# gylien/scale-letkf

Measured on AMD Instinct MI355X. Metric: grid-point LETKF solves/sec, higher is better.
Workload: dtype f64

## Files before the change

scale-letkf_amd/csrc/letkf_wave_dev.h:

```cpp
#pragma once
#include <hip/hip_runtime.h>
#include <stdint.h>

#include <type_traits>

#include "letkf_device.h"
#include "letkf_search_dev.h"
#include "letkf_jacobi_dev.h"
#include "letkf_lane_dev.h"
#include "letkf_sched_dev.h"

namespace letkf {

using namespace jacobi_dev;
using namespace lane_dev;

template <int NW, int OP>
__device__ __forceinline__ double preduce(double v, double* red, int& slot) {
  v = (OP == 0) ? wave_sum(v) : (OP == 1) ? wave_max(v) : wave_min(v);
  if constexpr (NW == 1) {
    return v;
  } else {
    if ((threadIdx.x & 63) == 0) red[2 * slot + (threadIdx.x >> 6)] = v;
    __syncthreads();
// ... 424 lines not shown
  if (NW == 1 && KR <= 50 && tot < 32 * KR + 64 * ((KR + 3) / 4) + 128)
    tot = 32 * KR + 64 * ((KR + 3) / 4) + 128;
  return (tot + 1) & ~1;
}

#ifdef LETKF_WAVE_PROF
#define PROF_DECL unsigned long long prof_t[10] = {0, 0, 0, 0, 0, 0, 0, 0, 0, 0}; unsigned long long prof_last = __builtin_amdgcn_s_memtime(); const unsigned long long prof_t0 = prof_last; int prof_units = 0;
#define PROF_MARK(i) { const unsigned long long t_ = __builtin_amdgcn_s_memtime(); prof_t[i] += t_ - prof_last; prof_last = t_; }
#define PROF_FLUSH if (A.prof && wlane == 0) { for (int i_ = 0; i_ < 10; ++i_) atomicAdd(&A.prof[i_], prof_t[i_]); \
    atomicMax(&A.prof[10], ~prof_t0); atomicMax(&A.prof[11], (unsigned long long)__builtin_amdgcn_s_memtime()); \
    atomicAdd(&A.prof[12 + (prof_units < 11 ? prof_units : 11)], 1ull); atomicAdd(&A.prof[24], (unsigned long long)prof_units); }
#define PROF_UNIT ++prof_units;
#else
#define PROF_DECL
#define PROF_MARK(i)
#define PROF_FLUSH
#define PROF_UNIT
#endif

#ifdef LETKF_CHECKED
#define LETKF_CHECK(ok, code, val, lim) letkf_check_fail(A.prof, (ok), (code), (long)(val), (long)(lim))
__device__ __forceinline__ bool letkf_check_fail(unsigned long long* rec, const bool ok, const int code, const long val, const long lim) {
  if (!ok && rec && atomicCAS(&rec[0], 0ull, (unsigned long long)code) == 0ull) {
    rec[1] = blockIdx.x;
    rec[2] = (unsigned long long)val;
    rec[3] = (unsigned long long)lim;
  }
  return ok;
}
#else
#define LETKF_CHECK(ok, code, val, lim) true
#endif

template <int KR, int NV, bool KKOUT, int NW, int FUSED>
__global__ void __launch_bounds__(NW == 1 ? 256 : 128, wave_occupancy(KR, NW)) letkf_wave_kernel(const PointArgs A) {
  extern __shared__ __attribute__((aligned(16))) double smem[];
  constexpr int NB = NV + 2;
  constexpr int NBP = (NB + 1) & ~1;
  constexpr int NL = 64 * NW;
  int lane = threadIdx.x & (NL - 1);
  int wlane = threadIdx.x & 63;
  const int wvp = (NW == 1) ? 0 : (threadIdx.x >> 6);
  const int wv = (NW == 1) ? (threadIdx.x >> 6) : 0;
  const int k = A.k;
  const int nv = A.nv;
  const double km1 = (double)(k - 1);

  double* slice = smem + (size_t)wv * wave_slice_doubles(KR, NV, NW);
  int tile_sz = kTnW * 64;
  if (KR * kVld > tile_sz) tile_sz = KR * kVld;
  int bmat_sz = NBP * KR;
  if (kChunk * KR > bmat_sz) bmat_sz = kChunk * KR;
  if (tile_sz + bmat_sz < wave_base_doubles(KR, NW)) bmat_sz = wave_base_doubles(KR, NW) - tile_sz;
  double* vbuf = slice;
  double* bmat = slice + tile_sz;
  double* cbuf = bmat + bmat_sz;
  double* wrow = cbuf + kChunk * NBP;
  double* xsm = wrow + 3 * kTnW;
  double* xmean = xsm;
  double* xdet = xsm + NV;
  double* red = xsm + 8 * NV + 16;
  int rslot = 0;

  constexpr int PPW = (NW == 1) ? 4 : 1;
  const int run_len = A.run_len;
  const long S = A.warm_stride, nA = A.npts / S;
  double* uws = (run_len > 1) ? A.warm_ws + ((size_t)blockIdx.x * PPW + wv) * ((size_t)KR * NL) + lane : nullptr;
  PROF_DECL
#ifdef LETKF_WAVE_PROF
  long Bstat = blockIdx.x;
#endif
  bool first_draw = true;
  int pend = 0;
  long next_rid = 0;
  for (;;) {
   long rid;
   int ir0 = 0, ir1 = run_len;
#ifdef LETKF_WAVE_PROF
   if (!A.sched) {
     const long nruns = S * ((nA + run_len - 1) / run_len);
     const long nB = (nruns + PPW - 1) / PPW;
     if (Bstat >= nB) break;
     rid = xcd_remap(Bstat, nB) * PPW + wv;
     Bstat += gridDim.x;
     if (rid >= nruns) continue;
   } else
#endif
   if (pend > 0) {
     rid = next_rid++;
     --pend;
   } else {
     int code;
     const int slot0 = first_draw ? (int)(blockIdx.x >> 3) * PPW + wv : -1;
     if constexpr (NW == 1) {
       code = sched_next(A.plan, A.sched, (int)(blockIdx.x & 7), slot0);
     } else {
       int* slot_ = reinterpret_cast<int*>(red + 6);
       __syncthreads();
       if (threadIdx.x < 64) {
         const int g = sched_next(A.plan, A.sched, (int)(blockIdx.x & 7), slot0);
         if (threadIdx.x == 0) *slot_ = g;
       }
       __syncthreads();
       code = *slot_;
     }
     first_draw = false;
     PROF_MARK(9)
     if (code < 0) break;
     PROF_UNIT
     if (code & 4) {
       ir0 = (code & 3) * run_len >> 2;
       ir1 = ((code & 3) + 1) * run_len >> 2;
     }
     rid = (long)(code >> 3) * A.plan.ub;
     const long left = A.plan.nruns - rid;
     pend = (int)(left < A.plan.ub ? left : A.plan.ub) - 1;
     next_rid = rid + 1;
   }
   const long rchunk = rid / S, rb = rid - rchunk * S;
   const long ra0 = rchunk * run_len;
   bool have_u = false;
   [[maybe_unused]] int pre_n = -1;
   for (int ir = ir0; ir < ir1; ++ir) {
    if (ra0 + ir >= nA) break;
    long pt = (ra0 + ir) * S + rb;
    if constexpr (FUSED == 3) {
      if (A.pt_stride) pt = (ra0 + ir) * A.pt_stride + rb + A.pt0;
    }
    if constexpr (NW == 2) asm volatile("" : "+v"(lane), "+v"(wlane));
    long o0 = 0;
    int n = 0;
    double beta = 1.0;
    const bool das = A.mode != 1;
    if (A.mode == 0) {
      o0 = A.obs_off[pt];
      n = (int)(A.obs_off[pt + 1] - o0);
      if (A.beta) beta = A.beta[pt];
    } else if (FUSED == 3 && A.mode == 3) {
      if (A.beta) beta = A.beta[pt];
      n = 0;
      if constexpr (NW == 1 && FUSED == 3) {
        if (pre_n >= 0) {
          o0 = ((long)blockIdx.x * PPW + wv) * (2 * A.sl_cap) + A.sl_cap;
          n = LETKF_CHECK(pre_n <= A.sl_cap, 7, pre_n, A.sl_cap) ? pre_n : 0;
          pre_n = -1;
        } else if (beta != 0.0) {
          using namespace search_dev;
          const letkf_search_tables& t = A.stab;
          o0 = ((long)blockIdx.x * PPW + wv) * (2 * A.sl_cap);
          const long o1 = o0 + A.sl_cap;
          const bool two = ir + 1 < ir1 && ra0 + ir + 1 < nA;
          const long ptn = two ? pt + (A.pt_stride ? A.pt_stride : S) : pt;
          const double v_z = A.prz[pt], v_p = log(A.prlev[pt]), l_rain = log(t.rain_base);
          const double v_z1 = A.prz[ptn], v_p1 = log(A.prlev[ptn]);
          const unsigned long long lt_mask = (wlane == 0) ? 0ull : (~0ull >> (64 - wlane));
          long s_lo = A.sv_off[rb], s_hi = A.sv_off[rb + 1];
#ifdef LETKF_CHECKED
          {
            bool ok = LETKF_CHECK(rb >= 0 && rb < S, 1, rb, S);
            ok = ok && LETKF_CHECK(s_hi >= s_lo && ((s_hi - s_lo) & 63) == 0, 2, s_hi - s_lo, 64);
            ok = ok && LETKF_CHECK(s_hi - s_lo <= A.sl_cap, 3, s_hi - s_lo, A.sl_cap);
            ok = ok && LETKF_CHECK((long)blockIdx.x < (long)A.wave_grid, 4, blockIdx.x, A.wave_grid);
            if (!ok) s_hi = s_lo;
          }
#endif
          int ntot = 0, ntot1 = 0;
          if (s_hi > s_lo) {
            const int ns_col = (int)(s_hi - s_lo);
            const double* sbase = A.surv + 4 * s_lo;
            int wl = wlane;
            asm volatile("" : "+v"(wl));
            auto ld = [&](const int e0, double2& x, double2& y) {
              int e = e0 + wl;
              e = e < ns_col ? e : ns_col - 1;
              x = *reinterpret_cast<const double2*>(&sbase[4 * e]);
              y = *reinterpret_cast<const double2*>(&sbase[4 * e + 2]);
            };
            double2 a0, b0, a1, b1, a2, b2, a3, b3;
            ld(0, a0, b0);
            ld(64, a1, b1);
            ld(128, a2, b2);
            ld(192, a3, b3);
            int ic_s = -1, vm_s = 0;
            double vloc_s = 0.0, varloc_s = 0.0;
            auto eval = [&](const double2& ca, const double2& cb, const bool live) {
              const long rw = __double_as_longlong(ca.x);
              const int ic0 = __builtin_amdgcn_readfirstlane((int)(rw >> 32));
              if (ic0 != ic_s) {
                ic_s = ic0;
                vm_s = t.vmode[ic0];
                vloc_s = t.vert_loc[ic0];
                varloc_s = t.varloc[ic0];
              }
              {
                const ColVert vo = column_vertical_cal(vm_s, vloc_s, varloc_s, ca.y, cb.x, cb.y, v_z, v_p, l_rain);
                const bool acc_ = live && vo.rloc != 0.0;
                const unsigned long long mk = __ballot(acc_);
                if (acc_ && LETKF_CHECK(ntot + __popcll(mk) <= A.sl_cap, 5, ntot + __popcll(mk), A.sl_cap)) {
                  const long j = o0 + ntot + __popcll(mk & lt_mask);
                  A.sl_idx[j] = (int)(rw & 0xffffffffL);
                  A.sl_rd[j] = vo.rdiag;
                  A.sl_rl[j] = vo.rloc;
                }
                ntot += __popcll(mk);
              }
              if (two) {
                const ColVert vo = column_vertical_cal(vm_s, vloc_s, varloc_s, ca.y, cb.x, cb.y, v_z1, v_p1, l_rain);
                const bool acc_ = live && vo.rloc != 0.0;
                const unsigned long long mk = __ballot(acc_);
                if (acc_ && LETKF_CHECK(ntot1 + __popcll(mk) <= A.sl_cap, 6, ntot1 + __popcll(mk), A.sl_cap)) {
                  const long j = o1 + ntot1 + __popcll(mk & lt_mask);
                  A.sl_idx[j] = (int)(rw & 0xffffffffL);
                  A.sl_rd[j] = vo.rdiag;
                  A.sl_rl[j] = vo.rloc;
                }
                ntot1 += __popcll(mk);
              }
            };
            for (int g0 = 0; g0 < ns_col; g0 += 256) {
              eval(a0, b0, true);
              ld(g0 + 256, a0, b0);
              eval(a1, b1, g0 + 64 < ns_col);
              ld(g0 + 320, a1, b1);
              eval(a2, b2, g0 + 128 < ns_col);
              ld(g0 + 384, a2, b2);
              eval(a3, b3, g0 + 192 < ns_col);
              ld(g0 + 448, a3, b3);
            }
          }
          if (two) pre_n = ntot1;
          n = ntot;
        }
      }
    } else if (FUSED == 2 && A.mode == 2) {
      n = -1;
      if (A.beta) beta = A.beta[pt];
    } else {
      n = A.nobsl[pt];
    }
    if (A.skip_trivial && (n == 0 || beta == 0.0)) {
      if (beta != 0.0) have_u = false;
      continue;
    }
    long moff = (long)lane * A.sm;
    asm volatile("" : "+v"(moff));
    const double* g0 = A.gues ? A.gues + pt * A.sp : nullptr;
    double* a0 = A.anal ? A.anal + pt * A.sp : nullptr;

    if (das && beta == 0.0) {
      for (int v = 0; v < nv; ++v) {
        if (lane < k && ((A.var_mask >> v) & 1u)) a0[moff + v * A.sv] = g0[k * A.sm + v * A.sv] + g0[moff + v * A.sv];
      }
      const bool mine = lane < nv && ((A.var_mask >> lane) & 1u);
      if (A.det_run && mine) a0[(k + 1) * A.sm + lane * A.sv] = g0[(k + 1) * A.sm + lane * A.sv];
      if (A.rtps_out && mine) A.rtps_out[pt + A.infl_sv * (long)lane] = 1.0;
      if (lane == 0) {
        if (A.status) A.status[pt] = 0;
        if (A.nsweep) A.nsweep[pt] = 0;
        if (A.nobs_out) A.nobs_out[pt] = 0;
      }
      continue;
    }

    bool qskip = false;
    if (das && A.q_update_top > 0.0) qskip = g0[k * A.sm + A.iv_p * A.sv] < A.q_update_top;
    int v0 = 0;
    while (v0 < nv && (!((A.var_mask >> v0) & 1u) || (qskip && v0 >= A.iv_q_first && v0 <= A.iv_q_last))) ++v0;
    double* infl_p = das ? ((v0 < nv) ? &A.infl[pt + A.infl_sv * (long)v0] : nullptr) : &A.infl[pt];
    const double infl_old = infl_p ? *infl_p : 1.0;

    PROF_MARK(0)
    double g[KR];
    double racc = 0.0, rdacc = 0.0, p1 = 0.0, p3 = 0.0;
    int sweeps = 0, jconv = 1;
    double lam = km1 / infl_old;
    bool colvalid = lane < k;

    bool solved = false;
    if (n != 0) {
      constexpr int NBLK = (KR + 2 + 15) / 16;
      constexpr int KMIN = (NW == 1) ? wave_kmin(KR, NW) : 1;
#ifndef LETKF_GRAM_STRIP
#define LETKF_GRAM_STRIP 1
#endif
      constexpr bool STRIP = LETKF_GRAM_STRIP && NW == 1 && (KR == 50 || KR == 20);
      constexpr int NBF = STRIP ? NBLK - 1 : NBLK;
      constexpr int RS = STRIP ? KR - 16 * (NBLK - 1) : 1;
      static_assert(!STRIP || (RS >= 1 && RS <= 6 && KMIN > 16 * (NBLK - 1)), "the narrow block must be the last one for every k of the instantiation");
      constexpr int NTILE = NBF * (NBF + 1) / 2;
      v4d acc[NTILE];
      [[maybe_unused]] double accS[RS][NBLK], accD[NBLK], accDD[NBLK], accP = 0.0;
#pragma unroll
      for (int I = 0; I < NBLK; ++I) accD[I] = accDD[I] = 0.0;
#pragma unroll
      for (int t = 0; t < NTILE; ++t) acc[t] = v4d{0.0, 0.0, 0.0, 0.0};
#pragma unroll
      for (int a = 0; a < RS; ++a)
#pragma unroll
        for (int I = 0; I < NBLK; ++I) accS[a][I] = 0.0;
      int q = wlane >> 4, c16 = wlane & 15;
      asm volatile("" : "+v"(q), "+v"(c16));

      constexpr int kSC = 256;
      double* stg = slice;
      const bool mode0 = A.mode != 1;
      const double* ybase = mode0 ? A.ensval : A.hdxb;
      bool rowok[NBLK];
      long mo[NBLK];
#pragma unroll
      for (int I = 0; I < NBLK; ++I) {
        const int m = 16 * I + c16;
        rowok[I] = m < k;
        const long mm = rowok[I] ? m : 0;
        mo[I] = mode0 ? mm : mm * (long)A.nobs;
      }
      const bool is_d = c16 == (k & 15), is_dd = c16 == ((k + 1) & 15);
      const int blk_d = k >> 4, blk_dd = (k + 1) >> 4;
      struct Step {
        double f[NBLK];
        double sw, dsw, ddsw;
      };

      auto run_steps = [&](const int nsp) {
        const int nch = nsp >> 2;
        auto fetch = [&](const int c, Step& t) {
          const bool ok = c < nch;
          const int i = 4 * (ok ? c : 0) + q;
          const double2 a2 = *reinterpret_cast<const double2*>(&stg[4 * i]);
          const double2 b2 = *reinterpret_cast<const double2*>(&stg[4 * i + 2]);
          const long rb = __double_as_longlong(a2.x);
          t.sw = ok ? a2.y : 0.0;
          t.dsw = ok ? b2.x : 0.0;
          t.ddsw = ok ? b2.y : 0.0;
#pragma unroll
          for (int I = 0; I < NBLK; ++I) t.f[I] = ybase[rb + mo[I]];
        };
        auto mma = [&](const Step& t) {
          double y[NBLK];
#pragma unroll
          for (int I = 0; I < NBLK; ++I) {
            double v = t.f[I] * t.sw;
            if (16 * (I + 1) > KMIN && 16 * (I + 1) > k) {
              v = rowok[I] ? v : 0.0;
              if constexpr (!STRIP) {
                if (I == blk_d && is_d) v = t.dsw;
                if (I == blk_dd && is_dd) v = t.ddsw;
              }
            }
            y[I] = v;
          }
          if constexpr (STRIP) {
#pragma unroll
            for (int I = 0; I < NBLK; ++I) {
              accD[I] = fma(y[I], t.dsw, accD[I]);
              accDD[I] = fma(y[I], t.ddsw, accDD[I]);
            }
            accP = fma(t.dsw, t.dsw, accP);
          }
          int tt = 0;
#pragma unroll
          for (int I = 0; I < NBF; ++I)
#pragma unroll
            for (int J = I; J < NBF; ++J) {
              acc[tt] = __builtin_amdgcn_mfma_f64_16x16x4f64(y[I], y[J], acc[tt], 0, 0, 0);
              ++tt;
            }
          if constexpr (STRIP) {
            auto strip_row = [&](auto a_) {
              constexpr int a = decltype(a_)::value;
              if constexpr (a < RS) {
#pragma unroll
                for (int I = 0; I < NBLK; ++I) {
                  if (a == 0 && I == 0) fmac_row_bcast<a, true>(accS[a][I], y[NBLK - 1], y[I]);
                  else fmac_row_bcast<a, false>(accS[a][I], y[NBLK - 1], y[I]);
                }
              }
            };
            strip_row(std::integral_constant<int, 0>{});
            strip_row(std::integral_constant<int, 1>{});
            strip_row(std::integral_constant<int, 2>{});
            strip_row(std::integral_constant<int, 3>{});
            strip_row(std::integral_constant<int, 4>{});
            strip_row(std::integral_constant<int, 5>{});
          }
        };
        if constexpr (NW == 1) {
          constexpr int PD = kGramDepth;
          Step ts[PD];
#pragma unroll
          for (int u = 0; u < PD; ++u) {
            fetch(wvp + u * NW, ts[u]);
            asm volatile("" ::: "memory");
          }
          auto pin = [&](Step& t) {
#pragma unroll
            for (int I = 0; I < NBLK; ++I) asm volatile("" : "+v"(t.f[I])::"memory");
          };
          for (int c = wvp; c < nch; c += PD * NW) {
#pragma unroll
            for (int u = 0; u < PD; ++u) {
              pin(ts[u]);
              if (u == 0 || c + u * NW < nch) mma(ts[u]);
              fetch(c + (PD + u) * NW, ts[u]);
            }
          }
        } else {
          Step t0, t1, t2;
          fetch(wvp, t0);
          fetch(wvp + NW, t1);
          fetch(wvp + 2 * NW, t2);
          for (int c = wvp; c < nch; c += 3 * NW) {
            mma(t0);
            fetch(c + 3 * NW, t0);
            if (c + NW < nch) {
              mma(t1);
              fetch(c + 4 * NW, t1);
            }
            if (c + 2 * NW < nch) {
              mma(t2);
              fetch(c + 5 * NW, t2);
            }
          }
        }
      };

      if (FUSED == 2 && A.mode == 2) {
        if constexpr (NW == 1 && FUSED == 2) {
          using namespace search_dev;
          const letkf_search_tables& t = A.stab;
          const double ri = A.pri[pt], rj = A.prj[pt], rlev = A.prlev[pt], rz = A.prz[pt];
          const unsigned long long lt_mask = (wlane == 0) ? 0ull : (~0ull >> (64 - wlane));
          int cnt = 0, ntot = 0, nconv = 0;
          auto convert = [&]() {
            for (int i = nconv + wlane; i < cnt; i += 64) {
              const double2 a2 = *reinterpret_cast<const double2*>(&stg[4 * i]);
              const double rloc_ = stg[4 * i + 2];
              const long row = __double_as_longlong(a2.x);
              const long rb = row * A.kld;
              const double d = A.dep[row];
              const double dd = A.det_run ? A.ensval[rb + k] : 0.0;
              const double sw = fast_rsqrt(a2.y);
              p3 += rloc_;
              *reinterpret_cast<double2*>(&stg[4 * i]) = double2{__longlong_as_double(rb), sw};
              *reinterpret_cast<double2*>(&stg[4 * i + 2]) = double2{d * sw, dd * sw};
            }
          };
          struct Meta {
            double lev, dat, ori, orj, err;
          };
          psync<NW>();
          for (int m = 0; m < t.group_start[t.ngroup]; ++m) {
            const int ic = t.group_member[m];
            const int vm = t.vmode[ic];
            const double dzi = t.hori_loc[ic] * kDistZeroFac / t.dx;
            const double dzj = t.hori_loc[ic] * kDistZeroFac / t.dy;
            int imin, imax, jmin, jmax;
            ij_obsgrd_ext(t, ic, ri - dzi, rj - dzj, imin, jmin);
            ij_obsgrd_ext(t, ic, ri + dzi, rj + dzj, imax, jmax);
            imin = max(imin, 1);
            jmin = max(jmin, 1);
            imax = min(imax, t.ngrdext_i[ic]);
            jmax = min(jmax, t.ngrdext_j[ic]);
            if (imin > imax || jmin > jmax) continue;
            const long acb = t.ac_off[ic];
            const int ld = t.ngrdext_i[ic] + 1;
            auto load_meta = [&](const int base, const int hi) -> Meta {
              Meta q_{1.0, 1.0, 0.0, 0.0, 1.0};
              const int row = base + wlane;
              if (row < hi) {
                if (vm != 2 && vm != 3) q_.lev = t.ob_lev[row];
                if (vm == 2) q_.dat = t.ob_dat[row];
                q_.ori = t.ob_ri[row];
                q_.orj = t.ob_rj[row];
                q_.err = t.ob_err[row];
              }
              return q_;
            };
            for (int j0 = jmin; j0 <= jmax; j0 += 64) {
              const int nr = min(64, jmax - j0 + 1);
              int lo_l = 0, hi_l = 0;
              if (wlane < nr) {
                lo_l = t.ac_ext[acb + (imin - 1) + (long)ld * (j0 + wlane - 1)];
                hi_l = t.ac_ext[acb + imax + (long)ld * (j0 + wlane - 1)];
              }
              int r = 0;
              int base = __shfl(lo_l, 0, 64), hi = __shfl(hi_l, 0, 64);
              auto skip_empty = [&]() {
                while (r < nr && base >= hi) {
                  ++r;
                  if (r < nr) {
                    base = __shfl(lo_l, r, 64);
                    hi = __shfl(hi_l, r, 64);
                  }
                }
              };
              skip_empty();
              Meta cur{1.0, 1.0, 0.0, 0.0, 1.0};
              if (r < nr) cur = load_meta(base, hi);
              while (r < nr) {
                const int cb = base, chi = hi;
                base += 64;
                skip_empty();
                Meta nxt{1.0, 1.0, 0.0, 0.0, 1.0};
                if (r < nr) nxt = load_meta(base, hi);
                const int row = cb + wlane;
                CalOut c{0.0, -1.0, -1.0};
                if (row < chi) c = local_cal_v(t, ic, ri, rj, rlev, rz, cur.lev, cur.dat, cur.ori, cur.orj, cur.err);
                const bool acc_ = c.rloc != 0.0;
                const unsigned long long mk = __ballot(acc_);
                if (acc_) {
                  const int i = cnt + __popcll(mk & lt_mask);
                  *reinterpret_cast<double2*>(&stg[4 * i]) = double2{__longlong_as_double((long)row), c.rdiag};
                  stg[4 * i + 2] = c.rloc;
                }
                const int na = __popcll(mk);
                cnt += na;
                ntot += na;
                if (cnt > kSC - 64) {
                  const int nuse = cnt & ~3;
                  psync<NW>();
                  convert();
                  psync<NW>();
                  run_steps(nuse);
                  psync<NW>();
                  double2 l0{0.0, 0.0}, l1{0.0, 0.0};
                  if (wlane < cnt - nuse) {
                    l0 = *reinterpret_cast<const double2*>(&stg[4 * (nuse + wlane)]);
                    l1 = *reinterpret_cast<const double2*>(&stg[4 * (nuse + wlane) + 2]);
                  }
                  psync<NW>();
                  if (wlane < cnt - nuse) {
                    *reinterpret_cast<double2*>(&stg[4 * wlane]) = l0;
                    *reinterpret_cast<double2*>(&stg[4 * wlane + 2]) = l1;
                  }
                  cnt -= nuse;
                  nconv = cnt;
                }
                cur = nxt;
              }
            }
          }
          psync<NW>();
          convert();
          const int nsp = (cnt + 3) & ~3;
          if (wlane < nsp - cnt) {
            *reinterpret_cast<double2*>(&stg[4 * (cnt + wlane)]) = double2{0.0, 0.0};
            *reinterpret_cast<double2*>(&stg[4 * (cnt + wlane) + 2]) = double2{0.0, 0.0};
          }
          psync<NW>();
          if (nsp > 0) run_steps(nsp);
          n = ntot;
        }
      } else
      for (int s0 = 0; s0 < n; s0 += kSC) {
        const int ns = min(kSC, n - s0);
        const int nsp = (ns + 3) & ~3;
        psync<NW>();
        constexpr int NPASS = kSC / NL;
        int iob[NPASS];
        double rdv[NPASS], rlv[NPASS], dv[NPASS], ddv[NPASS];
#pragma unroll
        for (int ps = 0; ps < NPASS; ++ps) {
          const int i = ps * NL + lane;
          iob[ps] = 0;
          rdv[ps] = 1.0;
          rlv[ps] = 0.0;
          dv[ps] = 0.0;
          ddv[ps] = 0.0;
          if (i < ns) {
            if (mode0) {
              const long e = o0 + s0 + i;
              iob[ps] = A.obs_idx[e];
              rlv[ps] = A.rloc_l[e];
              rdv[ps] = A.rdiag_l[e];
            } else {
              const long e = pt * (long)A.nobs + s0 + i;
              rlv[ps] = A.rloc[e];
              rdv[ps] = A.rdiag[e];
              dv[ps] = A.depv[e];
              if (A.depd) ddv[ps] = A.depd[e];
            }
          }
        }
        if (mode0) {
#pragma unroll
          for (int ps = 0; ps < NPASS; ++ps) {
            const int i = ps * NL + lane;
            if (i < ns) {
              dv[ps] = A.dep[iob[ps]];
              if (A.det_run) ddv[ps] = A.ensval[(long)iob[ps] * A.kld + k];
            }
          }
        }
#pragma unroll
        for (int ps = 0; ps < NPASS; ++ps) {
          const int i = ps * NL + lane;
          if (i < nsp) {
            double sw = 0.0;
            long rb = 0;
            if (i < ns) {
              sw = fast_rsqrt(rdv[ps]);
              if (!mode0 && !A.rdiag_wloc) sw *= sqrt(rlv[ps]);
              rb = mode0 ? (long)iob[ps] * A.kld : pt * (long)A.nobs * (long)k + (s0 + i);
              p3 += rlv[ps];
            }
            *reinterpret_cast<double2*>(&stg[4 * i]) = double2{__longlong_as_double(rb), sw};
            *reinterpret_cast<double2*>(&stg[4 * i + 2]) = double2{dv[ps] * sw, ddv[ps] * sw};
          }
        }
        psync<NW>();
        run_steps(nsp);
      }
      PROF_MARK(1)
      if (n > 0) {
      solved = true;
      constexpr int LDA = 18;
      double* abuf = slice;
      if constexpr (STRIP) {
#pragma unroll
        for (int a = 0; a < RS; ++a)
#pragma unroll
          for (int I = 0; I < NBLK; ++I) {
            accS[a][I] += wshfl_xor(accS[a][I], 16);
            accS[a][I] += wshfl_xor(accS[a][I], 32);
          }
#pragma unroll
        for (int I = 0; I < NBLK; ++I) {
          accD[I] += wshfl_xor(accD[I], 16);
          accD[I] += wshfl_xor(accD[I], 32);
          accDD[I] += wshfl_xor(accDD[I], 16);
          accDD[I] += wshfl_xor(accDD[I], 32);
        }
        accP += wshfl_xor(accP, 16);
        accP += wshfl_xor(accP, 32);
        racc = rdacc = 0.0;
#pragma unroll
        for (int I = 0; I < NBLK; ++I)
          if (q == I) {
            racc = accD[I];
            rdacc = accDD[I];
          }
        p1 = accP;
      }
#pragma unroll
      for (int I = 0; I < NBLK; ++I) {
        psync<NW>();
#pragma unroll
        for (int pass = 0; pass < NW; ++pass) {
          if (pass == 1) __syncthreads();
          if (wvp == pass) {
            if constexpr (STRIP) {
              {
                if (I < NBLK - 1) {
#pragma unroll
                  for (int a = 0; a < 16; ++a) abuf[(16 * (NBLK - 1) + a) * LDA + c16] = a < RS ? accS[a][I] : 0.0;
                } else {
#pragma unroll
                  for (int J = 0; J < NBLK; ++J)
#pragma unroll
                    for (int a = 0; a < RS; ++a) abuf[(16 * J + c16) * LDA + a] = accS[a][J];
                }
              }
            }
#pragma unroll
            for (int J = 0; J < NBF; ++J) {
              if (STRIP && I == NBLK - 1) continue;
              const int ti = I <= J ? I : J, tj = I <= J ? J : I;
              const int t = ti * NBF - ti * (ti - 1) / 2 + (tj - ti);
#pragma unroll
              for (int reg = 0; reg < 4; ++reg) {
                const int a = q + 4 * reg, b = c16;
                double* dst = (I <= J) ? &abuf[(16 * J + b) * LDA + a] : &abuf[(16 * J + a) * LDA + b];
                if (pass == 0) *dst = acc[t][reg];
                else *dst += acc[t][reg];
              }
            }
          }
        }
        psync<NW>();
        if constexpr (NW == 1) {
          const int lrow = lane < 16 * NBLK ? lane : 16 * NBLK - 1;
          const bool mine = lane < 16 * NBLK;
#pragma unroll
          for (int e = 0; e < 16; e += 2) {
            if (16 * I + e < KR) {
              const double2 v2 = *reinterpret_cast<const double2*>(&abuf[lrow * LDA + e]);
              g[16 * I + e] = v2.x;
              g[16 * I + e + 1] = v2.y;
            }
          }
          if constexpr (!STRIP) {
            if ((k >> 4) == I) {
              const double t = abuf[lrow * LDA + (k & 15)];
              racc = mine ? t : racc;
            }
            if (((k + 1) >> 4) == I) {
              const double t = abuf[lrow * LDA + ((k + 1) & 15)];
              rdacc = mine ? t : rdacc;
            }
          }
        } else if (lane < 16 * NBLK) {
#pragma unroll
          for (int e = 0; e < 16; e += 2) {
            if (16 * I + e < KR) {
              const double2 v2 = *reinterpret_cast<const double2*>(&abuf[lane * LDA + e]);
              g[16 * I + e] = v2.x;
              g[16 * I + e + 1] = v2.y;
            }
          }
          if constexpr (!STRIP) {
            if ((k >> 4) == I) racc = abuf[lane * LDA + (k & 15)];
            if (((k + 1) >> 4) == I) rdacc = abuf[lane * LDA + ((k + 1) & 15)];
          }
        }
        if constexpr (!STRIP) {
          if ((k >> 4) == I) p1 = abuf[k * LDA + (k & 15)];
        }
      }
      psync<NW>();
#pragma unroll
      for (int r = 0; r < KR; ++r)
        if (r >= k || lane >= k || lane >= 16 * NBLK) g[r] = 0.0;
      const double shift = km1 / infl_old;
      double diag = 0.0;
#pragma unroll
      for (int r = 0; r < KR; ++r) {
        if (r == lane && lane < k) {
          diag = g[r];
          g[r] += shift;
        }
      }
      double parm1 = 0.0, parm2 = 0.0, parm3 = 0.0;
      if (A.infl_adaptive) {
        parm1 = p1;
        parm3 = preduce<NW, 0>(p3, red, rslot);
        parm2 = preduce<NW, 0>(lane < k ? diag : 0.0, red, rslot) / km1;
      }

      PROF_MARK(2)
      if (have_u && !(A.warm_dbg & 1)) {
        if constexpr (LETKF_WARM_STRIP && NW == 1 && KR == 50) warm_start_product_strip<KR>(g, uws - lane, slice);
        else if constexpr (NW == 1 && KR <= 50) warm_start_product_mfma<KR>(g, uws - lane, slice);
        else warm_start_product<KR, NW>(g, uws, k, slice);
      }
      PROF_MARK(3)
      sweeps = jacobi_split<KR, NW, wave_jacobi_rc(KR, NW), true, LETKF_INPLACE_NW(KR, NW)>(g, k, A.max_sweep, slice, nullptr, &jconv);
      asm volatile("" : "+v"(racc), "+v"(rdacc), "+v"(moff));
      PROF_MARK(4)

      double ss = 0.0;
#pragma unroll
      for (int r = 0; r < KR; ++r) ss = fma(g[r], g[r], ss);
      lam = sqrt(ss);
      colvalid = ss > 0.0;
      const double il = colvalid ? 1.0 / lam : 0.0;
#pragma unroll
      for (int r = 0; r < KR; ++r) g[r] *= il;

      if (A.infl_adaptive) {
        const double parm4 = (parm1 - parm3) / parm2 - infl_old;
        const double tq = (infl_old * parm2 + parm3) / parm2;
        const double sigma_o = 2.0 / parm3 * (tq * tq);
        const double gain = 0.04 * 0.04 / (sigma_o + 0.04 * 0.04);
        p1 = infl_old + gain * parm4;
      }
      }
    }
    constexpr bool MAPPLY = !KKOUT && NW == 1 && KR <= 50 && NV > 0 && NB <= 14;
    constexpr int kBmRows = 4 * ((KR + 3) / 4), kBmOff = 32 * KR;
    constexpr int kObOff = (32 * KR >= 1024) ? 0 : kBmOff + 16 * kBmRows + 128;
    if constexpr (!MAPPLY) {
      if (!solved) {
#pragma unroll
        for (int r = 0; r < KR; ++r) g[r] = (r == lane && lane < k) ? 1.0 : 0.0;
      }
    }
    const double infl_new = (A.infl_adaptive && n > 0) ? p1 : infl_old;
    double xv[NV > 0 ? NV : 1];
    double xm_l = 0.0, xd_l = 0.0;
    if constexpr (MAPPLY) {
      const double* gp = g0 + moff;
#pragma unroll
      for (int v = 0; v < NV; ++v) {
        xv[v] = (lane < k) ? *gp : 0.0;
        gp += A.sv;
      }
      if (lane < NV) {
        xm_l = g0[k * A.sm + lane * A.sv];
        xd_l = A.det_run ? g0[(k + 1) * A.sm + lane * A.sv] : 0.0;
      }
      asm volatile("" ::: "memory");
    }
    {
      if (uws && solved && !(A.warm_dbg & 2)) {
        unsigned long long pa = reinterpret_cast<unsigned long long>(uws);
        if constexpr (LETKF_WARM_SORT && NW == 1) {
          int rk = warm_rank<KR>(lam, colvalid, lane);
          if constexpr (LETKF_WARM_ORDER) {
            const int nvalid = __popcll(__ballot(colvalid && lane < (KR < 64 ? KR : 64)));
            if (lane < (KR < 64 ? KR : 64) && !(A.warm_dbg & 32)) rk = warm_position(rk, nvalid);
          }
          pa += (long long)(((A.warm_dbg & 16) ? lane : rk) - lane) * (long long)sizeof(double);
        }
#pragma unroll
        for (int r = 0; r < KR; ++r) {
          if ((r & 7) == 0) asm volatile("" : "+v"(pa));
          ((gdouble*)pa)[(size_t)(r & 7) * NL] = g[r];
          if ((r & 7) == 7) pa += 8 * NL * sizeof(double);
        }
      }
    }

    int st = 0;
    {
      const double lmx = preduce<NW, 1>(colvalid ? lam : 0.0, red, rslot);
      const double lmn = preduce<NW, 2>(colvalid ? lam : 1e300, red, rslot);
      if (!jconv && A.max_sweep >= 60) st = 1;
      else if (!(lmx > 0.0)) st = 2;
      else if (lmn < lmx * 1.4901161193847656e-08) st = 3;
    }
    have_u = uws != nullptr && st == 0 && solved;
    const double sc1 = colvalid ? sqrt(km1 / lam) : 0.0;
    const double sc2 = colvalid ? 1.0 / lam : 0.0;

    PROF_MARK(5)
    const int mrow_l = lane < KR ? lane : KR - 1;
    double cf[NV > 0 ? NV : 1];
    double out[NB];
    if constexpr (MAPPLY) {
      if (!solved) {
        out[0] = 0.0;
        out[1] = 0.0;
        wave_lds_sync();
        if (lane < kBmRows) {
#pragma unroll
          for (int v = 0; v < NV; ++v) slice[kBmOff + lane * 16 + 2 + v] = xv[v];
        }
        wave_lds_sync();
#pragma unroll
        for (int v = 0; v < NV; ++v) {
          out[2 + v] = sc1 * xv[v];
          double cfv = 1.0;
          if (A.relax_alpha != 0.0) {
            cfv = 1.0 - A.relax_alpha;
          } else if (A.relax_alpha_spread != 0.0) {
            const double parm = A.relax_to_inflated_prior ? A.infl[pt + A.infl_sv * (long)v] : 1.0;
            const double var_g = wave_sum(xv[v] * xv[v]);
            const double var_a = var_g * uniform(sc2);
            if (var_g > 0.0 && var_a > 0.0)
              cfv = A.relax_alpha_spread * sqrt(var_g * parm / (var_a * km1)) - A.relax_alpha_spread + 1.0;
          }
          cf[v] = uniform(cfv);
          if (A.rtps_out && lane == 0 && ((A.var_mask >> v) & 1u)) {
            const bool skipv = qskip && v >= A.iv_q_first && v <= A.iv_q_last;
            A.rtps_out[pt + A.infl_sv * (long)v] = (A.relax_alpha == 0.0 && A.relax_alpha_spread != 0.0 && !skipv) ? cfv : 1.0;
          }
        }
      } else {
      constexpr int KS = (KR + 3) / 4;
      constexpr int BR = 4 * KS;
      double* vh = slice;
      double* bm = slice + 32 * KR;
      double* scl = bm + BR * 16;
      int q = wlane >> 4, c = wlane & 15;
      asm volatile("" : "+v"(q), "+v"(c));
      wave_lds_sync();
      {
        if (lane < BR) {
          double brow[16];
          brow[0] = (lane < k) ? racc : 0.0;
          brow[1] = (lane < k) ? rdacc : 0.0;
#pragma unroll
          for (int b = 2; b < 16; ++b) brow[b] = (b - 2 < NV) ? xv[b - 2 < NV ? b - 2 : 0] : 0.0;
          double* row = bm + lane * 16;
#pragma unroll
          for (int b = 0; b < 16; b += 2) *reinterpret_cast<double2*>(&row[b]) = double2{brow[b], brow[b + 1]};
        }
        *reinterpret_cast<double2*>(&scl[2 * lane]) = double2{sc2, sc1};
      }
      v4d accO[4];
#pragma unroll
      for (int t = 0; t < 4; ++t) accO[t] = v4d{0.0, 0.0, 0.0, 0.0};
      double va = 0.0, vg = 0.0;
#pragma unroll
      for (int h = 0; h < 2; ++h) {
        if (32 * h < KR) {
          wave_lds_sync();
          if ((lane >> 5) == h && lane < KR) {
            double* mine = vh + (lane - 32 * h) * KR;
#pragma unroll
            for (int r = 0; r < KR; r += 2) *reinterpret_cast<double2*>(&mine[r]) = double2{g[r], g[r + 1]};
          }
          wave_lds_sync();
          v4d accU[2];
          accU[0] = v4d{0.0, 0.0, 0.0, 0.0};
          accU[1] = v4d{0.0, 0.0, 0.0, 0.0};
#pragma unroll
          for (int s_ = 0; s_ < KS; ++s_) {
            const double bq = bm[(4 * s_ + q) * 16 + c];
            if (h == 0) vg = fma(bq, bq, vg);
#pragma unroll
            for (int il = 0; il < 2; ++il) {
              if (32 * h + 16 * il < KR) {
                const double a = vh[(16 * il + c) * KR + 4 * s_ + q];
                accU[il] = __builtin_amdgcn_mfma_f64_16x16x4f64(a, bq, accU[il], 0, 0, 0);
              }
            }
          }
#pragma unroll
          for (int il = 0; il < 2; ++il) {
#pragma unroll
            for (int reg = 0; reg < 4; ++reg) {
              const int s_ = 4 * (2 * h + il) + reg;
              if (4 * s_ < KR) {
                const int j = 4 * s_ + q;
                const double2 sc = *reinterpret_cast<const double2*>(&scl[2 * j]);
                const double u = accU[il][reg];
                va = fma(u * u, sc.x, va);
                const double cv = u * (c < 2 ? sc.x : sc.y);
                const double* a = vh + (j - 32 * h) * KR + 4 * c;
                const double2 lo = *reinterpret_cast<const double2*>(a);
                const double2 hi = *reinterpret_cast<const double2*>(a + 2);
                accO[0] = __builtin_amdgcn_mfma_f64_16x16x4f64(lo.x, cv, accO[0], 0, 0, 0);
                accO[1] = __builtin_amdgcn_mfma_f64_16x16x4f64(lo.y, cv, accO[1], 0, 0, 0);
                accO[2] = __builtin_amdgcn_mfma_f64_16x16x4f64(hi.x, cv, accO[2], 0, 0, 0);
                accO[3] = __builtin_amdgcn_mfma_f64_16x16x4f64(hi.y, cv, accO[3], 0, 0, 0);
              }
            }
          }
        }
      }
      PROF_MARK(6)
      va += wshfl_xor(va, 16);
      va += wshfl_xor(va, 32);
      vg += wshfl_xor(vg, 16);
      vg += wshfl_xor(vg, 32);
      {
        const int v = c - 2;
        const bool isv = c >= 2 && c < NB;
        double cfv = 1.0;
        if (A.relax_alpha != 0.0) {
          cfv = 1.0 - A.relax_alpha;
        } else if (A.relax_alpha_spread != 0.0) {
          const double parm = (A.relax_to_inflated_prior && isv) ? A.infl[pt + A.infl_sv * (long)v] : 1.0;
          if (vg > 0.0 && va > 0.0) cfv = A.relax_alpha_spread * sqrt(vg * parm / (va * km1)) - A.relax_alpha_spread + 1.0;
        }
        if (A.rtps_out && q == 0 && isv && ((A.var_mask >> v) & 1u)) {
          const bool skipv = qskip && v >= A.iv_q_first && v <= A.iv_q_last;
          A.rtps_out[pt + A.infl_sv * (long)v] = (A.relax_alpha == 0.0 && A.relax_alpha_spread != 0.0 && !skipv) ? cfv : 1.0;
        }
#pragma unroll
        for (int vv = 0; vv < NV; ++vv) cf[vv] = readlane_d(cfv, 2 + vv);
      }
      wave_lds_sync();
      double* ob = slice + kObOff;
      constexpr int OBR = wave_ob_rows(KR);
#pragma unroll
      for (int I = 0; I < 4; ++I)
#pragma unroll
        for (int reg = 0; reg < 4; ++reg)
          if (16 * reg < OBR) ob[(16 * reg + 4 * q + I) * 16 + c] = accO[I][reg];
      wave_lds_sync();
      {
        const double* row = ob + (OBR == 64 || lane < OBR ? lane : OBR - 1) * 16;
#pragma unroll
        for (int b = 0; b < NB; b += 2) {
          const double2 o2 = *reinterpret_cast<const double2*>(&row[b]);
          out[b] = o2.x;
          if (b + 1 < NB) out[b + 1] = o2.y;
        }
      }
      wave_lds_sync();
      }
    } else {
      psync<NW>();
      if (lane < KR) {
        bmat[lane * NBP + 0] = (lane < k) ? racc : 0.0;
        bmat[lane * NBP + 1] = (lane < k) ? rdacc : 0.0;
        if (NBP > NB) bmat[lane * NBP + NB] = 0.0;
      }
      if (NV > 0) {
        const double* gp = g0 + moff;
  #pragma unroll
        for (int v = 0; v < NV; ++v) {
          const double x = (lane < k) ? *gp : 0.0;
          gp += A.sv;
          if (lane < KR) bmat[lane * NBP + 2 + v] = x;
        }
        if (lane < NV) {
          xmean[lane] = g0[k * A.sm + lane * A.sv];
          xdet[lane] = A.det_run ? g0[(k + 1) * A.sm + lane * A.sv] : 0.0;
        }
      }
      psync<NW>();
      double crow[NB];
  #pragma unroll
      for (int b = 0; b < NB; ++b) crow[b] = 0.0;
  #pragma unroll
      for (int r = 0; r < KR; ++r) {
  #pragma unroll
        for (int b = 0; b < NBP; b += 2) {
          const double2 b2 = *reinterpret_cast<const double2*>(&bmat[r * NBP + b]);
          crow[b] = fma(g[r], b2.x, crow[b]);
          if (b + 1 < NB) crow[b + 1] = fma(g[r], b2.y, crow[b + 1]);
        }
        if ((r & 1) == 1) pin_acc<NB>(crow);
      }
      PROF_MARK(6)
      if (NV > 0) {
  #pragma unroll
        for (int v = 0; v < NV; ++v) {
          double cfv = 1.0;
          if (A.relax_alpha != 0.0) {
            cfv = 1.0 - A.relax_alpha;
          } else if (A.relax_alpha_spread != 0.0) {
            const double parm = A.relax_to_inflated_prior ? A.infl[pt + A.infl_sv * (long)v] : 1.0;
            const double x = (lane < k) ? bmat[mrow_l * NBP + 2 + v] : 0.0;
            const double var_g = preduce<NW, 0>(x * x, red, rslot);
            const double var_a = preduce<NW, 0>(crow[2 + v] * crow[2 + v] * sc2, red, rslot);
            if (var_g > 0.0 && var_a > 0.0)
              cfv = A.relax_alpha_spread * sqrt(var_g * parm / (var_a * km1)) - A.relax_alpha_spread + 1.0;
          }
          cf[v] = uniform(cfv);
          if (A.rtps_out && lane == 0 && ((A.var_mask >> v) & 1u)) {
            const bool skipv = qskip && v >= A.iv_q_first && v <= A.iv_q_last;
            A.rtps_out[pt + A.infl_sv * (long)v] = (A.relax_alpha == 0.0 && A.relax_alpha_spread != 0.0 && !skipv) ? cfv : 1.0;
          }
        }
      }
      crow[0] *= sc2;
      crow[1] *= sc2;
  #pragma unroll
      for (int v = 0; v < NV; ++v) crow[2 + v] *= sc1;

      rows_times_c<KR, NB, NW>(g, crow, out, k, vbuf, cbuf);

    }
    PROF_MARK(7)
    if (NV > 0 && das) {
      double* ap = a0 + moff;
#pragma unroll
      for (int v = 0; v < NV; ++v) {
        const bool skip = qskip && v >= A.iv_q_first && v <= A.iv_q_last;
        double x, xm, xdt;
        if constexpr (MAPPLY) {
          const double xl = slice[kBmOff + (lane < kBmRows ? lane : kBmRows - 1) * 16 + 2 + v];
          x = (lane < k) ? xl : 0.0;
          xm = readlane_d(xm_l, v);
          xdt = readlane_d(xd_l, v);
        } else {
          x = (lane < k) ? bmat[mrow_l * NBP + 2 + v] : 0.0;
          xm = xmean[v];
          xdt = xdet[v];
        }
        const double sdot = preduce<NW, 0>(x * out[0], red, rslot);
        const double sdotd = A.det_run ? preduce<NW, 0>(x * out[1], red, rslot) : 0.0;
        double val;
        if (skip) {
          val = xm + x;
        } else {
          double cdv = 0.0;
          if (A.relax_alpha != 0.0) {
            const double parm = A.relax_to_inflated_prior ? A.infl[pt + A.infl_sv * (long)v] : 1.0;
            cdv = A.relax_alpha * sqrt(parm);
          }
          const double pert = cf[v] * out[2 + v] + cdv * x;
          val = xm + beta * (pert + sdot) + (1.0 - beta) * x;
          if (A.q_sprd_max > 0.0 && v == A.iv_q_first) {
            const double q_mean = preduce<NW, 0>(lane < k ? val : 0.0, red, rslot) / (double)k;
            const double dq = (lane < k) ? val - q_mean : 0.0;
            const double q_sprd = sqrt(preduce<NW, 0>(dq * dq, red, rslot) / km1) / q_mean;
            if (q_sprd > A.q_sprd_max) val = q_mean + dq * A.q_sprd_max / q_sprd;
          }
        }
        const bool inclass = (A.var_mask >> v) & 1u;
        if (lane < k && inclass) *ap = val;
        ap += A.sv;
        if (A.det_run && lane == 0 && inclass)
          a0[(k + 1) * A.sm + v * A.sv] = skip ? xdt : xdt + sdotd * beta;
      }
      if (A.infl_adaptive) {
#pragma unroll
        for (int v = 0; v < NV; ++v) {
          const bool skip = qskip && v >= A.iv_q_first && v <= A.iv_q_last;
          if (!skip && lane == 0 && ((A.var_mask >> v) & 1u)) A.infl[pt + A.infl_sv * (long)v] = infl_new;
        }
      }
    } else if (A.infl_adaptive && n > 0 && lane == 0) {
      A.infl[pt] = infl_new;
    }

    if (A.transm_out && lane < k) A.transm_out[(size_t)pt * k + lane] = out[0];
    if (A.transmd_out && lane < k) A.transmd_out[(size_t)pt * k + lane] = out[1];
    if (KKOUT && (A.trans_out || A.pa_out)) {
      #pragma unroll 1
      for (int which = 0; which < 2; ++which) {
        double* dst = which == 0 ? A.trans_out : A.pa_out;
        if (!dst) continue;
        dst += (size_t)pt * k * k;
        const double sc = which == 0 ? sc1 : sc2;
        double kk[KR];
#pragma unroll
        for (int r = 0; r < KR; ++r) kk[r] = 0.0;
        double* ckk = bmat;
        const int ncol = (k + 1) & ~1;
        for (int j0 = 0; j0 < ncol; j0 += kChunk) {
          psync<NW>();
          if (lane >= j0 && lane < j0 + kChunk) {
            const int jj = lane - j0;
#pragma unroll
            for (int r = 0; r < KR; ++r) {
              vbuf[r * kVld + jj] = g[r];
              ckk[jj * KR + r] = sc * g[r];
            }
          }
          psync<NW>();
          const int mrow = lane < KR ? lane : KR - 1;
          const int nj = min(kChunk, ncol - j0);
          for (int jj = 0; jj < nj; ++jj) {
            const double vv = vbuf[mrow * kVld + jj];
#pragma unroll
            for (int r = 0; r < KR; r += 2) {
              const double2 c2 = *reinterpret_cast<const double2*>(&ckk[jj * KR + r]);
              kk[r] = fma(vv, c2.x, kk[r]);
              kk[r + 1] = fma(vv, c2.y, kk[r + 1]);
            }
          }
        }
        psync<NW>();
        if (lane < k) {
          const double add = (which == 0 && A.add_wbar_to_trans) ? 1.0 : 0.0;
#pragma unroll
          for (int r = 0; r < KR; ++r)
            if (r < k) dst[(size_t)r * k + lane] = kk[r] + add * out[0];
        }
      }
    }
    PROF_MARK(8)
    if (lane == 0) {
      if (A.status) A.status[pt] = st;
      if (A.nsweep) A.nsweep[pt] = sweeps;
      if (A.nobs_out) A.nobs_out[pt] = n;
    }
   }
  }
  PROF_FLUSH
}

template <int KR, int NV, bool KKOUT, int NW, int FUSED = 0>
static hipError_t launch_wave(const PointArgs& a, int num_cu, hipStream_t st) {
  const size_t lds = (size_t)(NW == 1 ? 4 : 1) * wave_slice_doubles(KR, NV, NW) * sizeof(double);
  if (a.k < wave_kmin(KR, NW) || a.k > KR) return hipErrorInvalidValue;
  if (hipError_t e = lds_opt_in(&letkf_wave_kernel<KR, NV, KKOUT, NW, FUSED>, lds)) return e;
  int grid = a.wave_grid;
  if (a.sched) {
    const int occ = resident_blocks(&letkf_wave_kernel<KR, NV, KKOUT, NW, FUSED>, NW == 1 ? 256 : 128, lds, NW == 1 ? 2 : 1);
    const long res = (long)occ * num_cu;
    const long S = a.warm_stride > 1 ? a.warm_stride : 1, rl = a.run_len > 1 ? a.run_len : 1;
    const long nruns = S * ((a.npts / S + rl - 1) / rl);
    constexpr int PPW = NW == 1 ? 4 : 1;
    if (NW == 1 && nruns < 8 * res * PPW) {
      const long need = 8 * (((nruns + 7) / 8 + PPW - 1) / PPW);
      if (grid > need) grid = (int)need;
    } else if (grid > res) {
      grid = (int)res;
    }
  }
  PointArgs b = a;
  if (a.sched) {
    sched_make_plan(b.plan, a.npts, a.warm_stride, a.run_len, grid, NW == 1 ? 4 : 1, NW == 1 ? 128 * wave_occupancy(KR, NW) : 64);
    if (hipError_t e = sched_reset_counters(b.plan, a.sched, st)) return e;
  }
  hipLaunchKernelGGL((letkf_wave_kernel<KR, NV, KKOUT, NW, FUSED>), dim3(grid), dim3(NW == 1 ? 256 : 128), lds, st, b);
  return hipGetLastError();
}

#define LETKF_WAVE_CASE(KR, NW)                                                                                 \
  if (k <= (NW == 1 ? (KR < 62 ? KR : 62) : KR)) {                                                              \
    if constexpr (NW == 1) {                                                                                    \
      if (a.mode == 2) return launch_wave<KR, 11, false, NW, 2>(a, num_cu, st);                                 \
      if (a.mode == 3) return launch_wave<KR, 11, false, NW, 3>(a, num_cu, st);                                 \
    }                                                                                                           \
    if (a.mode != 1)                                                                                            \
      return kkout ? launch_wave<KR, 11, true, NW>(a, num_cu, st) : launch_wave<KR, 11, false, NW>(a, num_cu, st); \
    return launch_wave<KR, 0, true, NW>(a, num_cu, st);                                                         \
  }

}
```

Before: 10.14 million.

## Pad Gram staging tail to drop per-step bounds checks and strip narrow apply MFMA

Fills the staging buffer past the last chunk with harmless padding entries: row pointer set to a valid row, weights zero. The single-wave Gram fetch can then drop its per-step bounds select and clamp. Separately, for KR==50 the apply stage replaces the mostly empty last 16-row MFMA block (rows 48-49) with two scalar FMA dot products plus a cross-lane shuffle reduction. Both aim to cut wasted instructions in the hot loops, at the cost of extra padding writes and syncs and some added complexity.

```diff
diff --git a/scale-letkf_amd/csrc/letkf_wave_dev.h b/scale-letkf_amd/csrc/letkf_wave_dev.h
--- a/scale-letkf_amd/csrc/letkf_wave_dev.h
+++ b/scale-letkf_amd/csrc/letkf_wave_dev.h
@@ -750,6 +750,12 @@
       asm volatile("" : "+v"(q), "+v"(c16));
 
       constexpr int kSC = 256;
+#ifndef LETKF_GRAM_PAD
+#define LETKF_GRAM_PAD 1
+#endif
+      constexpr bool PAD = LETKF_GRAM_PAD && NW == 1;
+      constexpr int kPadEnt = PAD ? 4 * (2 * kGramDepth - 1) : 0;
+      static_assert(4 * (kSC + kPadEnt) <= wave_base_doubles(KR, NW) && kPadEnt <= 64, "the staging buffer and its padding lie in the tile + bmat region");
       double* stg = slice;
       const bool mode0 = A.mode != 1;
       const double* ybase = mode0 ? A.ensval : A.hdxb;
@@ -772,16 +778,28 @@
       auto run_steps = [&](const int nsp) {
         const int nch = nsp >> 2;
         auto fetch = [&](const int c, Step& t) {
-          const bool ok = c < nch;
-          const int i = 4 * (ok ? c : 0) + q;
-          const double2 a2 = *reinterpret_cast<const double2*>(&stg[4 * i]);
-          const double2 b2 = *reinterpret_cast<const double2*>(&stg[4 * i + 2]);
-          const long rb = __double_as_longlong(a2.x);
-          t.sw = ok ? a2.y : 0.0;
-          t.dsw = ok ? b2.x : 0.0;
-          t.ddsw = ok ? b2.y : 0.0;
-#pragma unroll
-          for (int I = 0; I < NBLK; ++I) t.f[I] = ybase[rb + mo[I]];
+          if constexpr (PAD) {
+            const int i = 4 * c + q;
+            const double2 a2 = *reinterpret_cast<const double2*>(&stg[4 * i]);
+            const double2 b2 = *reinterpret_cast<const double2*>(&stg[4 * i + 2]);
+            const long rb = __double_as_longlong(a2.x);
+            t.sw = a2.y;
+            t.dsw = b2.x;
+            t.ddsw = b2.y;
+#pragma unroll
+            for (int I = 0; I < NBLK; ++I) t.f[I] = ybase[rb + mo[I]];
+          } else {
+            const bool ok = c < nch;
+            const int i = 4 * (ok ? c : 0) + q;
+            const double2 a2 = *reinterpret_cast<const double2*>(&stg[4 * i]);
+            const double2 b2 = *reinterpret_cast<const double2*>(&stg[4 * i + 2]);
+            const long rb = __double_as_longlong(a2.x);
+            t.sw = ok ? a2.y : 0.0;
+            t.dsw = ok ? b2.x : 0.0;
+            t.ddsw = ok ? b2.y : 0.0;
+#pragma unroll
+            for (int I = 0; I < NBLK; ++I) t.f[I] = ybase[rb + mo[I]];
+          }
         };
         auto mma = [&](const Step& t) {
           double y[NBLK];
@@ -891,6 +909,13 @@
               p3 += rloc_;
               *reinterpret_cast<double2*>(&stg[4 * i]) = double2{__longlong_as_double(rb), sw};
               *reinterpret_cast<double2*>(&stg[4 * i + 2]) = double2{d * sw, dd * sw};
+            }
+          };
+          [[maybe_unused]] auto pad_tail = [&](const int from, const int to) {
+            const double rb0 = stg[0];
+            if (wlane < to - from) {
+              *reinterpret_cast<double2*>(&stg[4 * (from + wlane)]) = double2{rb0, 0.0};
+              *reinterpret_cast<double2*>(&stg[4 * (from + wlane) + 2]) = double2{0.0, 0.0};
             }
           };
           struct Meta {
@@ -969,6 +994,10 @@
                   psync<NW>();
                   convert();
                   psync<NW>();
+                  if constexpr (PAD) {
+                    pad_tail(cnt, nuse + kPadEnt);
+                    psync<NW>();
+                  }
                   run_steps(nuse);
                   psync<NW>();
                   double2 l0{0.0, 0.0}, l1{0.0, 0.0};
@@ -991,7 +1020,10 @@
           psync<NW>();
           convert();
           const int nsp = (cnt + 3) & ~3;
-          if (wlane < nsp - cnt) {
+          if constexpr (PAD) {
+            psync<NW>();
+            if (nsp > 0) pad_tail(cnt, nsp + kPadEnt);
+          } else if (wlane < nsp - cnt) {
             *reinterpret_cast<double2*>(&stg[4 * (cnt + wlane)]) = double2{0.0, 0.0};
             *reinterpret_cast<double2*>(&stg[4 * (cnt + wlane) + 2]) = double2{0.0, 0.0};
           }
@@ -1040,12 +1072,20 @@
             }
           }
         }
+        long rb0 = 0;
+        if constexpr (PAD) rb0 = mode0 ? (long)__builtin_amdgcn_readfirstlane(iob[0]) * A.kld : pt * (long)A.nobs * (long)k + s0;
+        if constexpr (PAD) {
+          if (lane < kPadEnt) {
+            *reinterpret_cast<double2*>(&stg[4 * (nsp + lane)]) = double2{__longlong_as_double(rb0), 0.0};
+            *reinterpret_cast<double2*>(&stg[4 * (nsp + lane) + 2]) = double2{0.0, 0.0};
+          }
+        }
 #pragma unroll
         for (int ps = 0; ps < NPASS; ++ps) {
           const int i = ps * NL + lane;
           if (i < nsp) {
             double sw = 0.0;
-            long rb = 0;
+            long rb = rb0;
             if (i < ns) {
               sw = fast_rsqrt(rdv[ps]);
               if (!mode0 && !A.rdiag_wloc) sw *= sqrt(rlv[ps]);
@@ -1305,6 +1345,10 @@
           }
         }
       } else {
+#ifndef LETKF_APPLY_USTRIP
+#define LETKF_APPLY_USTRIP 1
+#endif
+      constexpr bool USTRIP = LETKF_APPLY_USTRIP && KR == 50;
       constexpr int KS = (KR + 3) / 4;
       constexpr int BR = 4 * KS;
       double* vh = slice;
@@ -1343,16 +1387,33 @@
           v4d accU[2];
           accU[0] = v4d{0.0, 0.0, 0.0, 0.0};
           accU[1] = v4d{0.0, 0.0, 0.0, 0.0};
+          [[maybe_unused]] double ue[2] = {0.0, 0.0};
 #pragma unroll
           for (int s_ = 0; s_ < KS; ++s_) {
             const double bq = bm[(4 * s_ + q) * 16 + c];
             if (h == 0) vg = fma(bq, bq, vg);
 #pragma unroll
             for (int il = 0; il < 2; ++il) {
-              if (32 * h + 16 * il < KR) {
+              if (32 * h + 16 * il < KR && !(USTRIP && h == 1 && il == 1)) {
                 const double a = vh[(16 * il + c) * KR + 4 * s_ + q];
                 accU[il] = __builtin_amdgcn_mfma_f64_16x16x4f64(a, bq, accU[il], 0, 0, 0);
               }
+            }
+            if constexpr (USTRIP) {
+              if (h == 1) {
+                ue[0] = fma(vh[16 * KR + 4 * s_ + q], bq, ue[0]);
+                ue[1] = fma(vh[17 * KR + 4 * s_ + q], bq, ue[1]);
+              }
+            }
+          }
+          if constexpr (USTRIP) {
+            if (h == 1) {
+#pragma unroll
+              for (int e = 0; e < 2; ++e) {
+                ue[e] += wshfl_xor(ue[e], 16);
+                ue[e] += wshfl_xor(ue[e], 32);
+              }
+              accU[1][0] = q == 0 ? ue[0] : q == 1 ? ue[1] : 0.0;
             }
           }
 #pragma unroll
```

New measurement: 10.20 million (median of 6 runs). About the same (+0.6%).
